# jabhinav/RetinaNet-for-Table-Detection

Hardware: AMD Instinct MI355X
Metric: images/sec RetinaNet R50-FPN 800x1333 inference (higher is better)
Workload: dtype bf16; 1 GPU; ResNet50-FPN RetinaNet inference 800x1333 bf16 batch 8/GPU incl. decode+NMS (BASELINE.json configs[1]); batch_per_gpu=8, anchors_per_image=200700, parallelism=dp1 (images sharded, no collective), batches_in_flight=2

## Files before the change

retinanet-for-table-detection_amd/csrc/rtn_conv_halo8.hip:

```cpp
#include "rtn_internal.h"
#include "rtn_device.h"
#include "rtn_conv_epilogue.h"

#ifndef RTN_H8_ABLATE
#define RTN_H8_ABLATE 0
#endif

namespace {

#ifdef RTN_H8_STAMP
__device__ unsigned long long g_h8_stamps[2][64];
#define H8_STAMP(K_)                                                                                 \
    if (stamp_on) {                                                                                  \
        unsigned long long t_;                                                                       \
        asm volatile("s_memtime %0\n\ts_waitcnt lgkmcnt(0)" : "=s"(t_) :: "memory");                 \
        if (lane == 0 && stamp_n < 64) g_h8_stamps[grp][stamp_n] = t_;                               \
        ++stamp_n;                                                                                   \
    }
#else
#define H8_STAMP(K_)
#endif

typedef __attribute__((ext_vector_type(8))) __bf16 bf16x8;
typedef __attribute__((ext_vector_type(4))) float f32x4;

constexpr unsigned OOB = 0xFFFFFF00u;
constexpr int H8_THREADS = 512;
constexpr int H8_LDS = 160 * 1024;
constexpr unsigned B_STAGE = 32768, A_BASE = 3 * 32768, A_TOGGLE = 0x18000u ^ 0x20000u;

struct H8Group {
    const char* in;
    char* out;
    const char* res;
    const char* mask;
    unsigned in_bytes, out_bytes, res_bytes, mask_bytes;
    int Hin, Win, M, tile_begin;
    int in_row_stride_b;
    int in_img_pad_b;
    float inv_cells, inv_w;
};

struct H8Params {
    H8Group g[RTN_MAX_GROUPS];
    const char* w;
    const float* bias;
    unsigned w_bytes;
    int ngroups, ntiles;
    int N, Kbytes, KH, nchunk, pad_t, pad_l, relu, out_ld, pix_b;
    int res_ld, mask_ld, mask_pre;
    int ncb, S, gps, nitems, xcd;
    int kh_fast;
    float* slab;
    unsigned slab_slice_bytes;
    int slab_ld;
    float acc_scale, out_scale;
    int out_fp8;
};

typedef int i32x8 __attribute__((ext_vector_type(8)));
__device__ __forceinline__ void mma_fp8(f32x4& acc, const uint4& a0, const uint4& a1, const uint4& b0, const uint4& b1) {
    const i32x8 A = __builtin_shufflevector(__builtin_bit_cast(i32x4, a0), __builtin_bit_cast(i32x4, a1), 0, 1, 2, 3, 4, 5, 6, 7);
    const i32x8 B = __builtin_shufflevector(__builtin_bit_cast(i32x4, b0), __builtin_bit_cast(i32x4, b1), 0, 1, 2, 3, 4, 5, 6, 7);
    acc = __builtin_amdgcn_mfma_scale_f32_16x16x128_f8f6f4(A, B, acc, 0, 0, 0, 0x7f7f7f7f, 0, 0x7f7f7f7f);
}

template <int KW, int MI, bool STAGGER, int EPI, bool SPLIT, int NW = 8, int ES = 2>
__global__ __launch_bounds__(H8_THREADS, 2) void conv_halo8_kernel(const H8Params p) {
    static_assert(NW == 8 || (NW == 4 && !SPLIT), "the half-width instance: no column blocks / K slices");
    static_assert(ES == 2 || (ES == 1 && NW == 8 && EPI == 0 && !SPLIT), "the fp8 instance: full width, plain epilogue");
    constexpr int NBP = NW / 2;
    constexpr int R = 64 * MI;
    constexpr int TM = R - KW;
    constexpr unsigned ZERO_ROW = (unsigned)(R - 1) * 128u;
    extern __shared__ __attribute__((aligned(16))) char lds[];

    const int t = threadIdx.x, lane = t & 63;
    const int wave = __builtin_amdgcn_readfirstlane(t >> 6);
    const int grp = wave >> 2;
#ifdef RTN_H8_STAMP
    bool stamp_on = false, first_item = true;
    int stamp_n = 0;
#endif
    const int wm = wave >> 1, wn = wave & 1;
    const int lr = lane >> 3, sc = (lane & 7) ^ lr;
    const int lrow = lane & 15, kq = lane >> 4;
    const unsigned lds_base = (unsigned)(size_t)(__attribute__((address_space(3))) char*)lds;

    const int G = p.KH * p.nchunk;
    const int nchunk = p.nchunk;
    const i32x4 w_srd = make_srd(p.w, p.w_bytes);

    unsigned wrow_off[NBP];
#pragma unroll
    for (int d = 0; d < NBP; ++d) {
        const int P = d * 64 + wave * 8 + lr;
        const int nrow = NW == 8 ? (P >> 7) * 128 + 8 * (P & 15) + ((P >> 4) & 7) : (P >> 6) * 64 + 4 * (P & 15) + ((P >> 4) & 3);
        wrow_off[d] = (unsigned)nrow * (unsigned)p.Kbytes + (unsigned)sc * 16u;
    }
    const unsigned b_lane = (unsigned)((wn * (16 * NW) + lrow) * 128 + ((kq ^ (lrow & 7)) << 4));


    unsigned hbase[MI];
    int hiy[MI];
    i32x4 in_srd = w_srd;
    int st_Hin = 1, st_row_b = 0;
    auto stage_tile = [&](int T) {
        if (T >= p.ntiles) {
#pragma unroll
            for (int i = 0; i < MI; ++i) { hiy[i] = -(1 << 28); hbase[i] = 0; }
            return;
        }
        int gi = 0;
#pragma unroll
        for (int i = 1; i < RTN_MAX_GROUPS; ++i)
            if (i < p.ngroups && T >= p.g[i].tile_begin) gi = i;

        const H8Group& Gs = p.g[gi];
        const int m0 = (T - Gs.tile_begin) * TM;
        const int cells = Gs.Hin * Gs.Win;
        in_srd = make_srd(Gs.in, Gs.in_bytes);
        st_Hin = Gs.Hin;
        st_row_b = Gs.in_row_stride_b;
#pragma unroll
        for (int i = 0; i < MI; ++i) {
            const int h = (i * 8 + wave) * 8 + lr;
            const int f = m0 + h - p.pad_l;
            if (h < R - 1 && f >= 0 && f < Gs.M) {
                int b, rem, y, x;
                divmod24(f, cells, Gs.inv_cells, b, rem);
                divmod24(rem, Gs.Win, Gs.inv_w, y, x);
                hiy[i] = y;
                hbase[i] = (unsigned)f * (unsigned)p.pix_b + (unsigned)b * (unsigned)Gs.in_img_pad_b + (unsigned)sc * 16u;
            } else {
                hiy[i] = -(1 << 28);
                hbase[i] = 0;
            }
        }
    };
    auto stage_a = [&](int i, int kh, int cc, unsigned abuf_addr) {
        const int dy = kh - p.pad_t;
        const unsigned delta = (unsigned)(dy * st_row_b + cc * 128);
        const bool ok = (unsigned)(hiy[i] + dy) < (unsigned)st_Hin;
#if !(RTN_H8_ABLATE & 2)
        dma16(in_srd, ok ? hbase[i] + delta : OOB, 0u, lds_base + abuf_addr + (unsigned)(wave * 1024 + i * 8192));
#endif
    };
    auto stage_b = [&](int d, unsigned kcol, int bst) {
#if !(RTN_H8_ABLATE & 1)
        dma16(w_srd, wrow_off[d], kcol, lds_base + (unsigned)bst * B_STAGE + (unsigned)(wave * 1024 + d * 8192));
#endif
    };

    unsigned a_cur = A_BASE;
    unsigned arow[KW][MI];
    auto compute_tile = [&](int T, int& gi_out, int& m0_out) {
        int gi = 0;
#pragma unroll
        for (int i = 1; i < RTN_MAX_GROUPS; ++i)
            if (i < p.ngroups && T >= p.g[i].tile_begin) gi = i;
        const H8Group& Gc = p.g[gi];
        const int m0 = (T - Gc.tile_begin) * TM;
        const int cells = Gc.Hin * Gc.Win;
        gi_out = gi;
        m0_out = m0;
#pragma unroll
        for (int i = 0; i < MI; ++i) {
            const int rloc = wm * (16 * MI) + i * 16 + lrow;
            const int m = m0 + rloc;
            const int mc = m < Gc.M ? m : Gc.M - 1;
            int b, rem, y, x;
            divmod24(mc, cells, Gc.inv_cells, b, rem);
            divmod24(rem, Gc.Win, Gc.inv_w, y, x);
#pragma unroll
            for (int kw = 0; kw < KW; ++kw) {
                const int rr = rloc + kw;
                const bool off = rloc >= TM || (unsigned)(x + kw - p.pad_l) >= (unsigned)Gc.Win;
                arow[kw][i] = a_cur + (off ? ZERO_ROW : (unsigned)(rr * 128 + ((kq ^ (rr & 7)) << 4)));
            }
        }
    };

    f32x4 acc[MI][NW];
    float bias8[8];
#pragma unroll
    for (int j = 0; j < 8; ++j) bias8[j] = 0.f;
    if (!SPLIT && p.bias && wn * (16 * NW) + NW * lrow < p.N) {
        const float4 b0 = *reinterpret_cast<const float4*>(p.bias + wn * (16 * NW) + NW * lrow);
        bias8[0] = b0.x; bias8[1] = b0.y; bias8[2] = b0.z; bias8[3] = b0.w;
        if (NW == 8) {
            const float4 b1 = *reinterpret_cast<const float4*>(p.bias + wn * 128 + 8 * lrow + 4);
            bias8[4] = b1.x; bias8[5] = b1.y; bias8[6] = b1.z; bias8[7] = b1.w;
        }
    }

    auto item_of = [&](int v) {
        if (v >= p.nitems || !p.xcd) return v;
        const int x = v & 7, j = v >> 3, base = p.nitems >> 3, rem = p.nitems & 7;
        return x * base + (x < rem ? x : rem) + j;
    };
    auto item_decode = [&](int it, int& rt, int& cb, int& sl, unsigned& cboff, int& kh0, int& cc0) {
        if (!SPLIT || it >= p.nitems) { rt = it >= p.nitems ? p.ntiles : it; cb = 0; sl = 0; cboff = 0u; kh0 = 0; cc0 = 0; return; }
        const int per = p.ncb * p.S;
        rt = it / per;
        const int rem = it - rt * per;
        cb = rem / p.S;
        sl = rem - cb * p.S;
        cboff = (unsigned)cb * 256u * (unsigned)p.Kbytes;
        const int g0 = sl * p.gps;
        if (p.kh_fast) { cc0 = g0 / p.KH; kh0 = g0 - cc0 * p.KH; }
        else { kh0 = g0 / nchunk; cc0 = g0 - kh0 * nchunk; }
    };
    const int gps = SPLIT ? p.gps : G;

    int vidx = blockIdx.x;
    int rt, cb, sl, kh0, cc0;
    unsigned cboff;
    item_decode(item_of(vidx), rt, cb, sl, cboff, kh0, cc0);
    stage_tile(rt);
#pragma unroll
    for (int i = 0; i < MI; ++i) stage_a(i, kh0, cc0, A_BASE);
    {
        const unsigned kc0 = cboff + (unsigned)((kh0 * KW * nchunk + cc0) * 128);
#pragma unroll
        for (int d = 0; d < NBP; ++d) stage_b(d, kc0, 0);
#pragma unroll
        for (int d = 0; d < NBP - 1; ++d) stage_b(d, kc0 + (unsigned)(nchunk * 128), 1);
    }
    if (NW == 8) asm volatile("s_waitcnt vmcnt(3)" ::: "memory");
    else         asm volatile("s_waitcnt vmcnt(1)" ::: "memory");
    if (STAGGER && grp == 1) __builtin_amdgcn_s_barrier();
    __builtin_amdgcn_s_barrier();


#if RTN_H8_ABLATE & 8
#define H8_LDA(KWI, KS)                                                                              \
    _Pragma("unroll") for (int i_ = 0; i_ < MI; ++i_)                                                \
        asm volatile("" : "=v"(fa[i_].x), "=v"(fa[i_].y), "=v"(fa[i_].z), "=v"(fa[i_].w));
#define H8_LDB(KWI, KS, HALF)                                                                        \
    _Pragma("unroll") for (int j_ = 0; j_ < 4; ++j_)                                                 \
        asm volatile("" : "=v"(fb[j_].x), "=v"(fb[j_].y), "=v"(fb[j_].z), "=v"(fb[j_].w));
#else
#define H8_LDA(KWI, KS)                                                                              \
    _Pragma("unroll") for (int i_ = 0; i_ < MI; ++i_)                                                \
        fa[i_] = *reinterpret_cast<const uint4*>(lds + (arow[KWI][i_] ^ ((KS) * 64u)));
#define H8_LDB(KWI, KS, HALF)                                                                        \
    _Pragma("unroll") for (int j_ = 0; j_ < 4; ++j_)                                                 \
        fb[j_] = *reinterpret_cast<const uint4*>(lds + (b_lane ^ ((KS) * 64u)) + (KWI) * B_STAGE + ((HALF) * 4 + j_) * 2048);
#endif
#if RTN_H8_ABLATE & 4
#define H8_MMA(I_, J_, HALF) asm volatile("" :: "v"(fa[I_].x), "v"(fa[I_].w), "v"(fb[J_].x), "v"(fb[J_].w));
#else
#define H8_MMA(I_, J_, HALF)                                                                         \
    acc[I_][(HALF) * 4 + J_] = __builtin_amdgcn_mfma_f32_16x16x32_bf16(                              \
        __builtin_bit_cast(bf16x8, fa[I_]), __builtin_bit_cast(bf16x8, fb[J_]), acc[I_][(HALF) * 4 + J_], 0, 0, 0);
#endif
#define H8_MFMA(HALF)                                                                                \
    H8_STAMP(1)                                                                                      \
    __builtin_amdgcn_s_barrier();                                                                    \
    H8_STAMP(2)                                                                                      \
    __builtin_amdgcn_sched_barrier(0);                                                               \
    __builtin_amdgcn_s_setprio(1);                                                                   \
    _Pragma("unroll") for (int j_ = 0; j_ < 4; ++j_)                                                 \
        _Pragma("unroll") for (int i_ = 0; i_ < MI; ++i_)                                            \
            H8_MMA(i_, j_, HALF)                                                                     \
    __builtin_amdgcn_s_setprio(0);                                                                   \
    __builtin_amdgcn_sched_barrier(0);                                                               \
    H8_STAMP(3)                                                                                      \
    __builtin_amdgcn_s_barrier();                                                                    \
    H8_STAMP(4)
#define H8_STEP(KWI)                                                                                 \
    {                                                                                                \
        const unsigned kc_n1 = (KWI) + 1 < KW ? kcol_g + ((KWI) + 1) * kw_stride : kcol_g1;          \
        const unsigned kc_n2 = (KWI) + 2 < KW ? kcol_g + ((KWI) + 2) * kw_stride : kcol_g1 + ((KWI) + 2 - KW) * kw_stride; \
        uint4 fa[MI], fb[4];                                                                         \
                                                                                        \
        H8_LDA(KWI, 0) H8_LDB(KWI, 0, 0)                                                             \
        stage_b(3, kc_n1, ((KWI) + 1) % 3);                                                          \
        H8_MFMA(0)                                                                                   \
                                                                                        \
        H8_LDB(KWI, 0, 1)                                                                            \
        stage_b(0, kc_n2, ((KWI) + 2) % 3);                                                          \
        if (2 * (KWI) < MI && (KWI) < 2) stage_a(2 * (KWI), kh1, cc1, a_cur ^ A_TOGGLE);                 \
        H8_MFMA(1)                                                                                   \
                                                                                        \
        H8_LDA(KWI, 1) H8_LDB(KWI, 1, 0)                                                             \
        stage_b(1, kc_n2, ((KWI) + 2) % 3);                                                          \
        H8_MFMA(0)                                                                                   \
                                                                                        \
        H8_LDB(KWI, 1, 1)                                                                            \
        stage_b(2, kc_n2, ((KWI) + 2) % 3);                                                          \
        if (2 * (KWI) + 1 < MI && (KWI) < 2) stage_a(2 * (KWI) + 1, kh1, cc1, a_cur ^ A_TOGGLE);         \
         \
        {                                                                                            \
            constexpr int na_ = (KWI) < 2 ? ((2 * (KWI) < MI) + (2 * (KWI) + 1 < MI)) : 0;           \
            if (na_ == 2)      asm volatile("s_waitcnt vmcnt(5)" ::: "memory");                      \
            else if (na_ == 1) asm volatile("s_waitcnt vmcnt(4)" ::: "memory");                      \
            else               asm volatile("s_waitcnt vmcnt(3)" ::: "memory");                      \
        }                                                                                            \
        H8_MFMA(1)                                                                                   \
    }
#define H8_MFMA8(HALF)                                                                               \
    __builtin_amdgcn_s_barrier();                                                                    \
    __builtin_amdgcn_sched_barrier(0);                                                               \
    __builtin_amdgcn_s_setprio(1);                                                                   \
    _Pragma("unroll") for (int j_ = 0; j_ < 4; ++j_)                                                 \
        _Pragma("unroll") for (int i_ = 0; i_ < MI; ++i_)                                            \
            mma_fp8(acc[i_][(HALF) * 4 + j_], fa[i_], fa1[i_], fb[j_], fb1[j_]);                      \
    __builtin_amdgcn_s_setprio(0);                                                                   \
    __builtin_amdgcn_sched_barrier(0);                                                               \
    __builtin_amdgcn_s_barrier();
#define H8_STEP8F(KWI)                                                                               \
    {                                                                                                \
        const unsigned kc_n1 = (KWI) + 1 < KW ? kcol_g + ((KWI) + 1) * kw_stride : kcol_g1;          \
        const unsigned kc_n2 = (KWI) + 2 < KW ? kcol_g + ((KWI) + 2) * kw_stride : kcol_g1 + ((KWI) + 2 - KW) * kw_stride; \
        uint4 fa[MI], fa1[MI], fb[4], fb1[4];                                                        \
        H8_LDA(KWI, 0)                                                                               \
        _Pragma("unroll") for (int i_ = 0; i_ < MI; ++i_)                                            \
            fa1[i_] = *reinterpret_cast<const uint4*>(lds + (arow[KWI][i_] ^ 64u));                  \
        H8_LDB(KWI, 0, 0)                                                                            \
        _Pragma("unroll") for (int j_ = 0; j_ < 4; ++j_)                                             \
            fb1[j_] = *reinterpret_cast<const uint4*>(lds + (b_lane ^ 64u) + (KWI) * B_STAGE + j_ * 2048); \
        stage_b(3, kc_n1, ((KWI) + 1) % 3);                                                          \
        if (2 * (KWI) < MI && (KWI) < 2) stage_a(2 * (KWI), kh1, cc1, a_cur ^ A_TOGGLE);             \
        H8_MFMA8(0)                                                                                  \
        H8_LDB(KWI, 0, 1)                                                                            \
        _Pragma("unroll") for (int j_ = 0; j_ < 4; ++j_)                                             \
            fb1[j_] = *reinterpret_cast<const uint4*>(lds + (b_lane ^ 64u) + (KWI) * B_STAGE + (4 + j_) * 2048); \
        stage_b(0, kc_n2, ((KWI) + 2) % 3);                                                          \
        stage_b(1, kc_n2, ((KWI) + 2) % 3);                                                          \
        stage_b(2, kc_n2, ((KWI) + 2) % 3);                                                          \
        if (2 * (KWI) + 1 < MI && (KWI) < 2) stage_a(2 * (KWI) + 1, kh1, cc1, a_cur ^ A_TOGGLE);     \
        {                                                                                            \
            constexpr int na_ = (KWI) < 2 ? ((2 * (KWI) < MI) + (2 * (KWI) + 1 < MI)) : 0;           \
            if (na_ == 2)      asm volatile("s_waitcnt vmcnt(5)" ::: "memory");                      \
            else if (na_ == 1) asm volatile("s_waitcnt vmcnt(4)" ::: "memory");                      \
            else               asm volatile("s_waitcnt vmcnt(3)" ::: "memory");                      \
        }                                                                                            \
        H8_MFMA8(1)                                                                                  \
    }
#define H8_STEP4(KWI)                                                                                \
    {                                                                                                \
        const unsigned kc_n1 = (KWI) + 1 < KW ? kcol_g + ((KWI) + 1) * kw_stride : kcol_g1;          \
        const unsigned kc_n2 = (KWI) + 2 < KW ? kcol_g + ((KWI) + 2) * kw_stride : kcol_g1 + ((KWI) + 2 - KW) * kw_stride; \
        uint4 fa[MI], fb[4];                                                                         \
        H8_LDA(KWI, 0) H8_LDB(KWI, 0, 0)                                                             \
        stage_b(1, kc_n1, ((KWI) + 1) % 3);                                                          \
        if (2 * (KWI) < MI && (KWI) < 2) stage_a(2 * (KWI), kh1, cc1, a_cur ^ A_TOGGLE);             \
        H8_MFMA(0)                                                                                   \
        H8_LDA(KWI, 1) H8_LDB(KWI, 1, 0)                                                             \
        stage_b(0, kc_n2, ((KWI) + 2) % 3);                                                          \
        if (2 * (KWI) + 1 < MI && (KWI) < 2) stage_a(2 * (KWI) + 1, kh1, cc1, a_cur ^ A_TOGGLE);     \
        {                                                                                            \
            constexpr int na_ = (KWI) < 2 ? ((2 * (KWI) < MI) + (2 * (KWI) + 1 < MI)) : 0;           \
            if (na_ == 2)      asm volatile("s_waitcnt vmcnt(3)" ::: "memory");                      \
            else if (na_ == 1) asm volatile("s_waitcnt vmcnt(2)" ::: "memory");                      \
            else               asm volatile("s_waitcnt vmcnt(1)" ::: "memory");                      \
        }                                                                                            \
        H8_MFMA(0)                                                                                   \
    }
    static_assert(KW == 3 && MI >= 2 && MI <= 4, "the B ring (3 stages) and the halo piece slots are laid out for KW = 3, MI <= 4");

    const unsigned kw_stride = (unsigned)(nchunk * 128);
    while (rt < p.ntiles) {
        int gi, m0;
        compute_tile(rt, gi, m0);
#pragma unroll
        for (int i = 0; i < MI; ++i)
#pragma unroll
            for (int j = 0; j < NW; ++j) acc[i][j] = (SPLIT || ES == 1) ? (f32x4){0.f, 0.f, 0.f, 0.f} : (f32x4){bias8[j], bias8[j], bias8[j], bias8[j]};
        int kh = kh0, cc = cc0;
        int rt1 = rt, cb1 = cb, sl1 = sl;
        unsigned cboff1 = cboff;
#pragma unroll 1
        for (int g = 0; g < gps; ++g) {
            int kh1 = kh, cc1 = cc;
            if (p.kh_fast) { if (++kh1 == p.KH) { kh1 = 0; ++cc1; } }
            else if (++cc1 == nchunk) { cc1 = 0; ++kh1; }
            if (g + 1 == gps) {
                vidx += (int)gridDim.x;
                item_decode(item_of(vidx), rt1, cb1, sl1, cboff1, kh1, cc1);
                stage_tile(rt1);
            }
#ifdef RTN_H8_STAMP
            stamp_on = blockIdx.x == 0 && (wave & 3) == 0 && first_item && g == 4;
#endif
            const unsigned kcol_g = cboff + (unsigned)((kh * KW * nchunk + cc) * 128);
            const unsigned kcol_g1 = cboff1 + (unsigned)((kh1 * KW * nchunk + cc1) * 128);
            if constexpr (ES == 1) {
                H8_STEP8F(0)
                H8_STEP8F(1)
                H8_STEP8F(2)
            } else if constexpr (NW == 8) {
                H8_STEP(0)
                H8_STEP(1)
                H8_STEP(2)
            } else {
                H8_STEP4(0)
                H8_STEP4(1)
                H8_STEP4(2)
            }
#pragma unroll
            for (int kw = 0; kw < KW; ++kw)
#pragma unroll
                for (int i = 0; i < MI; ++i) arow[kw][i] ^= A_TOGGLE;
            a_cur ^= A_TOGGLE;
            kh = kh1; cc = cc1;
        }
        kh0 = kh; cc0 = cc;
        if constexpr (ES == 1) {
            const H8Group& Gc = p.g[gi];
            const __amdgpu_buffer_rsrc_t out_rsrc = epi_rsrc(Gc.out, Gc.out_bytes);
            const int ncol = wn * 128 + 8 * lrow;
            const bool col_ok = ncol < p.N;
#pragma unroll
            for (int i = 0; i < MI; ++i)
#pragma unroll
                for (int r = 0; r < 4; ++r) {
                    const int rloc = wm * (16 * MI) + i * 16 + kq * 4 + r;
                    const int m = m0 + rloc;
                    const bool ok = col_ok && rloc < TM && m < Gc.M;
                    float v[8];
#pragma unroll
                    for (int j = 0; j < 8; ++j) {
                        v[j] = acc[i][j][r] * p.acc_scale + bias8[j];
                        if (p.relu) v[j] = v[j] > 0.f ? v[j] : 0.f;
                    }
                    if (p.out_fp8) epi_store8(epi_quant_fp8(v, p.out_scale), out_rsrc, ok ? (unsigned)m * (unsigned)p.out_ld + (unsigned)ncol : OOB);
                    else epi_store_bf16<8>(v, out_rsrc, ok ? ((unsigned)m * (unsigned)p.out_ld + (unsigned)ncol) * 2u : OOB);
                }
        } else if (SPLIT && p.S > 1) {
            const __amdgpu_buffer_rsrc_t slab_rsrc = epi_rsrc((char*)p.slab + (size_t)sl * p.slab_slice_bytes, p.slab_slice_bytes);
            const int gcol = cb * 256 + wn * 128 + 8 * lrow;
            const int Mg = p.g[gi].M;
#pragma unroll
            for (int i = 0; i < MI; ++i)
#pragma unroll
                for (int r = 0; r < 4; ++r) {
                    const int rloc = wm * (16 * MI) + i * 16 + kq * 4 + r;
                    const int m = m0 + rloc;
                    const bool ok = gcol < p.slab_ld && rloc < TM && m < Mg;
                    const unsigned off = ok ? ((unsigned)m * (unsigned)p.slab_ld + (unsigned)gcol) * 4u : OOB;
                    epi_store_f32x8<0>(acc[i], r, slab_rsrc, off, ok ? off + 16u : OOB);
                }
        } else {
            const H8Group& Gc = p.g[gi];
            const __amdgpu_buffer_rsrc_t out_rsrc = epi_rsrc(Gc.out, Gc.out_bytes);
            const __amdgpu_buffer_rsrc_t res_rsrc = epi_rsrc(Gc.res, Gc.res_bytes, EPI & 1, Gc.out);
            const __amdgpu_buffer_rsrc_t mask_rsrc = epi_rsrc(Gc.mask, Gc.mask_bytes, EPI & 2, Gc.out);
            const int ncol = (SPLIT ? cb * 256 : 0) + wn * (16 * NW) + NW * lrow;
            const bool col_ok = ncol < p.N;
            float bias_e[8];
#pragma unroll
            for (int j = 0; j < 8; ++j) bias_e[j] = 0.f;
            if (SPLIT && p.bias && col_ok) {
                const float4 b0 = *reinterpret_cast<const float4*>(p.bias + ncol);
                const float4 b1 = *reinterpret_cast<const float4*>(p.bias + ncol + 4);
                bias_e[0] = b0.x; bias_e[1] = b0.y; bias_e[2] = b0.z; bias_e[3] = b0.w;
                bias_e[4] = b1.x; bias_e[5] = b1.y; bias_e[6] = b1.z; bias_e[7] = b1.w;
            }
            constexpr int EDEPTH = NW == 8 && (EPI == 3 || (EPI == 1 && MI == 4)) ? 2 : MI;
            u32x4 rq[EDEPTH][4], mq[EDEPTH][4];
            const unsigned res_ld = (unsigned)p.res_ld, mask_ld = (unsigned)p.mask_ld;
#pragma unroll
            for (int f = 0; f < MI + EDEPTH - 1; ++f) {
                if (EPI && f < MI) {
#pragma unroll
                    for (int r = 0; r < 4; ++r) {
                        const int rloc = wm * (16 * MI) + f * 16 + kq * 4 + r;
                        const int m = m0 + rloc;
                        const bool ok = col_ok && rloc < TM && m < Gc.M;
                        if (EPI & 1) rq[f % EDEPTH][r] = epi_load_row<NW>(res_rsrc, ok ? ((unsigned)m * res_ld + (unsigned)ncol) * 2u : OOB);
                        if (EPI & 2) mq[f % EDEPTH][r] = epi_load_row<NW>(mask_rsrc, ok ? ((unsigned)m * mask_ld + (unsigned)ncol) * 2u : OOB);
                    }
                }
                const int i = f - (EDEPTH - 1);
                if (i < 0) continue;
#pragma unroll
                for (int r = 0; r < 4; ++r) {
                    const int rloc = wm * (16 * MI) + i * 16 + kq * 4 + r;
                    const int m = m0 + rloc;
                    const bool ok = col_ok && rloc < TM && m < Gc.M;
                    const unsigned off = ok ? ((unsigned)m * (unsigned)p.out_ld + (unsigned)ncol) * 2u : OOB;
                    float v[NW];
#pragma unroll
                    for (int j = 0; j < NW; ++j) v[j] = NW == 8 ? acc[i][j][r] + (SPLIT ? bias_e[j] : 0.f) : acc[i][j][r];
                    if (EPI) epi_mask_res<NW, EPI>(v, rq[i % EDEPTH][r], mq[i % EDEPTH][r], p.mask_pre);
                    if (p.relu) epi_relu(v);
                    epi_store_bf16<NW>(v, out_rsrc, off);
                }
            }
        }
        rt = rt1; cb = cb1; sl = sl1; cboff = cboff1;
#ifdef RTN_H8_STAMP
        first_item = false;
#endif
    }
#undef H8_STEP4
#undef H8_STEP8F
#undef H8_MFMA8
#undef H8_STEP
#undef H8_MFMA
#undef H8_MMA
#undef H8_LDB
#undef H8_LDA
    asm volatile("s_waitcnt vmcnt(0)" ::: "memory");
    if (STAGGER && grp == 0) __builtin_amdgcn_s_barrier();
}

template <int MI, bool ST, int EP, bool SP, int NW = 8, int ES = 2>
int h8_go(rtn_handle_t h, int grid, const H8Params& p) {
    return rtn_launch_lds<conv_halo8_kernel<3, MI, ST, EP, SP, NW, ES>>(h, dim3((unsigned)grid), dim3(H8_THREADS), H8_LDS, H8_LDS, p);
}
template <int MI>
int h8_pick(rtn_handle_t h, int grid, const H8Params& p, bool fp8, bool half, bool split, bool stagger, int epi) {
    if (fp8) return h8_go<3, true, 0, false, 8, 1>(h, grid, p);
    if (half) return rtn_with_epi<3>(epi, [&](auto e) { return h8_go<MI, true, decltype(e)::value, false, 4>(h, grid, p); });
    if (split) return h8_go<MI, true, 0, true>(h, grid, p);
    if (!stagger && epi == 0) return h8_go<MI, false, 0, false>(h, grid, p);
    return rtn_with_epi<3>(epi, [&](auto e) { return h8_go<MI, true, decltype(e)::value, false>(h, grid, p); });
}
}

int rtn_conv_halo8_try(rtn_handle_t h, const rtn_conv_desc_t* d, int grid_limit, bool stagger, bool forced, int mi_force, float* ws,
                       long long ws_cap, size_t* query, int ksplit_force, const rtn_conv_fp8_t* q8) {
    if (query) *query = 0;
    if (q8 ? d->dtype != RTN_FP8 : d->dtype != RTN_BF16) return 1;
    const int es = q8 ? 1 : 2;
    if (q8 && (query || (d->flags & ~RTN_CONV_RELU) || d->N <= 128 || d->N > 256)) return 1;
    if (d->KW != 3 || d->KH < 1 || d->KH > 7 || d->sy != 1 || d->sx != 1) return 1;
    if (d->flags & ~(RTN_CONV_RELU | RTN_CONV_RES_SAME | RTN_CONV_RELU_MASK | RTN_CONV_MASK_PRE)) return 1;
    if ((d->flags & RTN_CONV_MASK_PRE) && !(d->flags & RTN_CONV_RELU_MASK)) return 1;
    const int epi = ((d->flags & RTN_CONV_RES_SAME) ? 1 : 0) | ((d->flags & RTN_CONV_RELU_MASK) ? 2 : 0);
    const int ncb = (d->N + 255) / 256;
    if (d->N <= 64 || ncb > 8 || d->w_rows < d->N || d->N % 8 || d->out_ld % 8) return 1;
    if (ncb > 1 && epi) return 1;
    const bool half = d->N <= 128;
    if (half && !forced && rtn_env_int("RTN_CONV_H8_HALF", 1) == 0) return 1;
    if (d->Crun != d->pix_stride || (d->Crun * es) % 128 || d->Crun <= 0) return 1;
    if (d->pad_l < 0 || d->pad_l >= d->KW || d->pad_t < 0 || d->pad_t >= d->KH) return 1;
    if (((uintptr_t)d->w & 15) || ((uintptr_t)d->bias & 15)) return 1;
    const int nchunk = d->Crun * es / 128;
    const int G = d->KH * nchunk;
    const long long Kbytes = (long long)d->KH * d->KW * d->Crun * es;
    if (Kbytes * 256 * ncb >= 0xFFFFFF00ll) return 1;
    H8Params p;
    memset(&p, 0, sizeof(p));
    const int cus = h->num_cus > 0 ? h->num_cus : 256;
    long long Mtot = 0;
    for (int i = 0; i < d->ngroups; ++i) Mtot += (long long)d->g[i].Hout * d->g[i].Wout * d->batch;
    const bool can_split = !half && !q8 && d->ngroups == 1 && epi == 0 && ksplit_force != 1 && (ws_cap > 0 || query);
    const long long slab_ld = 256ll * ncb;
    int mi = 0, S = 1;
    {
        double best = 0;
        for (int cand = 4; cand >= 3; --cand) {
            if (!q8 && mi_force >= 3 && mi_force <= 4 && cand != mi_force) continue;
            if (q8 && cand == 4) continue;
            long long t = 0;
            for (int i = 0; i < d->ngroups; ++i) t += ((long long)d->g[i].Hout * d->g[i].Wout * d->batch + 64 * cand - 4) / (64 * cand - 3);
            const double step_us = 1.53 * (cand + 0.3) / 4.3;
            for (int sc = 1; sc <= 8; ++sc) {
                if (sc > 1 && (!can_split || G % sc || (ksplit_force > 1 && sc != ksplit_force))) continue;
                if (sc == 1 && ksplit_force > 1 && can_split && G % ksplit_force == 0) continue;
                if (sc > 1 && (double)sc * Mtot * slab_ld * 4 > (double)(query ? (256ll << 20) : ws_cap)) continue;
                const long long items = t * ncb * sc;
                double cost = (double)((items + cus - 1) / cus) * (3.0 * G / sc + 5.0) * step_us;
                if (sc > 1) cost += 4.0 + ((double)sc * Mtot * slab_ld * 4 + (double)Mtot * d->N * 2) / 4.0e6;
                if (mi == 0 || cost < best * 0.97) { best = cost; mi = cand; S = sc; }
            }
        }
        if (mi == 0) return 1;
    }
    if (S > 1 && !query && (!ws || ((uintptr_t)ws & 15))) return 1;
    const bool split = ncb > 1 || S > 1;
    const int TM = 64 * mi - 3;
    long long tiles = 0;
    for (int i = 0; i < d->ngroups; ++i) {
        const rtn_conv_group_t& s = d->g[i];
        if (s.Hin != s.Hout || s.Win != s.Wout || s.in_row_stride != (long long)s.Win * d->pix_stride ||
            s.in_img_stride < (long long)s.Hin * s.in_row_stride) return 1;
        if (s.in_elems < (long long)(d->batch - 1) * s.in_img_stride + (long long)s.Hin * s.in_row_stride) return 1;
        const long long cells = (long long)s.Hout * s.Wout, M = cells * d->batch;
        if (s.out_step > 1 || s.out_off != 0 || s.out_img_stride != cells * d->out_ld) return 1;
        if (M >= (1ll << 24) || M < 1) return 1;
        if (!s.in || !s.out || ((uintptr_t)s.in & 15) || ((uintptr_t)s.out & 15)) return 1;
        if (s.in_elems < M * d->Crun || s.out_elems < (M - 1) * d->out_ld + d->N) return 1;
        if (s.in_elems * 2 >= 0xFFFFFF00ll || s.out_elems * 2 >= 0xFFFFFF00ll) return 1;
        if (epi & 1) {
            if (!s.res || ((uintptr_t)s.res & 15) || s.res_ld % 8 || s.res_img_stride != cells * s.res_ld) return 1;
            if (s.res_elems < (M - 1) * s.res_ld + d->N || s.res_elems * 2 >= 0xFFFFFF00ll) return 1;
        }
        if (epi & 2) {
            if (!s.mask || ((uintptr_t)s.mask & 15) || s.mask_ld % 8 || s.mask_img_stride != cells * s.mask_ld) return 1;
            if (s.mask_elems < (M - 1) * s.mask_ld + d->N || s.mask_elems * 2 >= 0xFFFFFF00ll) return 1;
        }
        if (i > 0 && ((epi & 1) && s.res_ld != d->g[0].res_ld)) return 1;
        if (i > 0 && ((epi & 2) && s.mask_ld != d->g[0].mask_ld)) return 1;
        H8Group& g = p.g[i];
        g.res = (epi & 1) ? (const char*)s.res : nullptr;
        g.mask = (epi & 2) ? (const char*)s.mask : nullptr;
        g.res_bytes = (epi & 1) ? (unsigned)(s.res_elems * 2) : 0u;
        g.mask_bytes = (epi & 2) ? (unsigned)(s.mask_elems * 2) : 0u;
        g.in = (const char*)s.in;
        g.out = (char*)s.out;
        g.in_bytes = (unsigned)(s.in_elems * es);
        g.out_bytes = (unsigned)(s.out_elems * ((q8 && q8->out_dtype == RTN_FP8) ? 1 : 2));
        g.Hin = s.Hin; g.Win = s.Win; g.M = (int)M;
        g.tile_begin = (int)tiles;
        g.in_row_stride_b = (int)(s.in_row_stride * es);
        g.in_img_pad_b = (int)((s.in_img_stride - (long long)s.Hin * s.in_row_stride) * es);
        g.inv_cells = 1.0f / (float)cells;
        g.inv_w = 1.0f / (float)s.Win;
        tiles += (M + TM - 1) / TM;
    }
    const long long items = tiles * ncb * S;
    if (tiles < 1 || items > 0x3fffffff) return 1;
    if (!forced && items * 4 < cus) return 1;
    const long long slice_bytes = Mtot * slab_ld * 4;
    if (S > 1 && slice_bytes >= 0xFFFFFF00ll) return 1;
    if (query) { *query = S > 1 ? (size_t)(slice_bytes * S) : 0; return RTN_OK; }
    p.w = (const char*)d->w;
    p.bias = d->bias;
    p.w_bytes = (unsigned)(Kbytes * d->w_rows);
    p.ngroups = d->ngroups;
    p.ntiles = (int)tiles;
    p.N = d->N;
    p.Kbytes = (int)Kbytes;
    p.KH = d->KH;
    p.nchunk = nchunk;
    p.pad_t = d->pad_t; p.pad_l = d->pad_l;
    p.relu = (d->flags & RTN_CONV_RELU) ? 1 : 0;
    p.out_ld = d->out_ld;
    p.pix_b = d->pix_stride * es;
    if (q8) { p.acc_scale = q8->acc_scale; p.out_scale = q8->out_scale; p.out_fp8 = q8->out_dtype == RTN_FP8 ? 1 : 0; }
    p.res_ld = (epi & 1) ? d->g[0].res_ld : 0;
    p.mask_ld = (epi & 2) ? d->g[0].mask_ld : 0;
    p.mask_pre = (d->flags & RTN_CONV_MASK_PRE) ? 1 : 0;
    p.ncb = ncb; p.S = S; p.gps = G / S; p.nitems = (int)items;
    p.xcd = 1;
    p.kh_fast = 1;
    p.slab = S > 1 ? ws : nullptr;
    p.slab_slice_bytes = S > 1 ? (unsigned)slice_bytes : 0u;
    p.slab_ld = (int)slab_ld;
    int grid = cus;
    if (grid_limit > 0 && grid_limit < grid) grid = grid_limit;
    if (grid > p.nitems) grid = p.nitems;
    const int lrc = mi == 4 ? h8_pick<4>(h, grid, p, q8 != nullptr, half, split, stagger, epi)
                            : h8_pick<3>(h, grid, p, q8 != nullptr, half, split, stagger, epi);
    if (lrc != RTN_OK) return lrc;
    RTN_CHECK_LAUNCH(h, "conv_halo8_kernel");
    h->last_conv_tile = ((64 * mi) << 16) | (half ? 128 : 256);
    if (S > 1) return rtn_conv_ksplit_finish(h, ws, S, Mtot, d->N, (int)slab_ld, d->bias, p.relu, d->g[0].out, d->out_ld);
    return RTN_OK;
}

#ifdef RTN_H8_STAMP
extern "C" int rtn_debug_h8_stamps(unsigned long long* out128) {
    return (int)hipMemcpyFromSymbol(out128, HIP_SYMBOL(g_h8_stamps), sizeof(unsigned long long) * 128, 0, hipMemcpyDeviceToHost);
}
#endif
```

Measured before the change: 2420 images/sec.

## Add warp-specialized split4 halo conv kernel for half-width N tiles

Adds a new 3x3 halo conv kernel for the half-N (128 columns, MI=3) case with no fused residual or mask epilogue. Four waves act as dedicated DMA producers staging weights and halo rows into LDS, and four waves run MFMA compute with double-buffered fragments interleaved by sched_group_barrier. It is enabled by default through an environment switch. The goal is to overlap global-to-LDS transfer with matrix math instead of having every wave do both. In exchange, only half the waves issue MFMAs, the kernel relies on hand-tuned vmcnt and barrier counts, and it serves only this tile shape.

After: 2441 images/sec, median of 6. No clear change (+0.8%).

```diff
diff --git a/retinanet-for-table-detection_amd/csrc/rtn_conv_halo8.hip b/retinanet-for-table-detection_amd/csrc/rtn_conv_halo8.hip
--- a/retinanet-for-table-detection_amd/csrc/rtn_conv_halo8.hip
+++ b/retinanet-for-table-detection_amd/csrc/rtn_conv_halo8.hip
@@ -508,13 +508,289 @@
     if (STAGGER && grp == 0) __builtin_amdgcn_s_barrier();
 }
 
+__global__ __launch_bounds__(H8_THREADS, 2) void conv_halo8_split4_kernel(const H8Params p) {
+    constexpr int KW = 3, MI = 3, FM = 6, NW = 4;
+    constexpr int R = 64 * MI, TM = R - KW;
+    constexpr unsigned ZERO_ROW = (unsigned)(R - 1) * 128u;
+    extern __shared__ __attribute__((aligned(16))) char lds[];
+
+    const int t = threadIdx.x, lane = t & 63;
+    const int wave = __builtin_amdgcn_readfirstlane(t >> 6);
+    const unsigned lds_base = (unsigned)(size_t)(__attribute__((address_space(3))) char*)lds;
+    const int G = p.KH * p.nchunk, nchunk = p.nchunk;
+    const unsigned kw_stride = (unsigned)(nchunk * 128);
+    auto tile_of = [&](int v) {
+        if (v >= p.ntiles) return p.ntiles;
+        if (!p.xcd) return v;
+        const int x = v & 7, j = v >> 3, base = p.ntiles >> 3, rem = p.ntiles & 7;
+        return x * base + (x < rem ? x : rem) + j;
+    };
+    auto group_of = [&](int T) {
+        int gi = 0;
+#pragma unroll
+        for (int i = 1; i < RTN_MAX_GROUPS; ++i)
+            if (i < p.ngroups && T >= p.g[i].tile_begin) gi = i;
+        return gi;
+    };
+    const int ntile_wg = (p.ntiles - (int)blockIdx.x + (int)gridDim.x - 1) / (int)gridDim.x;
+
+    if (wave >= 4) {
+        const int sw = wave - 4;
+        const int lr = lane >> 3, sc = (lane & 7) ^ lr;
+        const i32x4 w_srd = make_srd(p.w, p.w_bytes);
+        unsigned wrow_off[2][2];
+#pragma unroll
+        for (int d = 0; d < 2; ++d)
+#pragma unroll
+            for (int u = 0; u < 2; ++u) {
+                const int P = d * 64 + (2 * sw + u) * 8 + lr;
+                const int nrow = (P >> 6) * 64 + 4 * (P & 15) + ((P >> 4) & 3);
+                wrow_off[d][u] = (unsigned)nrow * (unsigned)p.Kbytes + (unsigned)sc * 16u;
+            }
+        unsigned hbase[MI][2];
+        int hiy[MI][2];
+        const char* st_in = p.w;
+        unsigned st_in_bytes = 0;
+        int st_Hin = 1, st_row_b = 0;
+        auto stage_tile = [&](int T) {
+            if (T >= p.ntiles) {
+#pragma unroll
+                for (int i = 0; i < MI; ++i) { hiy[i][0] = hiy[i][1] = -(1 << 28); hbase[i][0] = hbase[i][1] = 0; }
+                return;
+            }
+            const H8Group& Gs = p.g[group_of(T)];
+            const int m0 = (T - Gs.tile_begin) * TM;
+            const int cells = Gs.Hin * Gs.Win;
+            st_in = Gs.in;
+            st_in_bytes = Gs.in_bytes;
+            st_Hin = Gs.Hin;
+            st_row_b = Gs.in_row_stride_b;
+#pragma unroll
+            for (int i = 0; i < MI; ++i)
+#pragma unroll
+                for (int u = 0; u < 2; ++u) {
+                    const int h = (i * 8 + 2 * sw + u) * 8 + lr;
+                    const int f = m0 + h - p.pad_l;
+                    if (h < R - 1 && f >= 0 && f < Gs.M) {
+                        int b, rem, y, x;
+                        divmod24(f, cells, Gs.inv_cells, b, rem);
+                        divmod24(rem, Gs.Win, Gs.inv_w, y, x);
+                        hiy[i][u] = y;
+                        hbase[i][u] = (unsigned)f * (unsigned)p.pix_b + (unsigned)b * (unsigned)Gs.in_img_pad_b + (unsigned)sc * 16u;
+                    } else {
+                        hiy[i][u] = -(1 << 28);
+                        hbase[i][u] = 0;
+                    }
+                }
+        };
+        int hv = blockIdx.x, hkh = 0, hcc = 0;
+        unsigned hbuf = A_BASE;
+        int bkh = 0, bcc = 0;
+        struct Cur { int kh, cc; bool left; };
+        auto next_group = [&](int kh, int cc) {
+            if (p.kh_fast) { if (++kh == p.KH) { kh = 0; ++cc; } }
+            else if (++cc == nchunk) { cc = 0; ++kh; }
+            const bool left = p.kh_fast ? cc == nchunk : kh == p.KH;
+            return Cur{left ? 0 : kh, left ? 0 : cc, left};
+        };
+        auto stage_halo = [&]() {
+            const int dy = hkh - p.pad_t;
+            const unsigned delta = (unsigned)(dy * st_row_b + hcc * 128);
+            const i32x4 srd = make_srd(st_in, st_in_bytes);
+#pragma unroll
+            for (int i = 0; i < MI; ++i)
+#pragma unroll
+                for (int u = 0; u < 2; ++u) {
+                    const bool ok = (unsigned)(hiy[i][u] + dy) < (unsigned)st_Hin;
+#if !(RTN_H8_ABLATE & 2)
+                    dma16_uniform(srd, ok ? hbase[i][u] + delta : OOB, 0u, lds_base + hbuf + (unsigned)((2 * sw + u) * 1024 + i * 8192));
+#endif
+                }
+            hbuf ^= A_TOGGLE;
+            const Cur n = next_group(hkh, hcc);
+            hkh = n.kh; hcc = n.cc;
+            if (n.left) { hv += (int)gridDim.x; stage_tile(tile_of(hv)); }
+        };
+        auto stage_b = [&](int kw) {
+            const unsigned kcol = (unsigned)__builtin_amdgcn_readfirstlane((int)((unsigned)((bkh * KW * nchunk + bcc) * 128) + (unsigned)kw * kw_stride));
+#pragma unroll
+            for (int d = 0; d < 2; ++d)
+#pragma unroll
+                for (int u = 0; u < 2; ++u) {
+#if !(RTN_H8_ABLATE & 1)
+                    dma16_uniform(w_srd, wrow_off[d][u], kcol, lds_base + (unsigned)kw * B_STAGE + (unsigned)((2 * sw + u) * 1024 + d * 8192));
+#endif
+                }
+        };
+        stage_tile(tile_of(hv));
+        stage_halo();
+        stage_b(0);
+        stage_b(1);
+        stage_b(2);
+        { const Cur n = next_group(bkh, bcc); bkh = n.kh; bcc = n.cc; }
+        stage_halo();
+        asm volatile("s_waitcnt vmcnt(14)" ::: "memory");
+        __builtin_amdgcn_s_barrier();
+#pragma unroll 1
+        for (int g = ntile_wg * G; g > 0; --g) {
+            asm volatile("s_waitcnt vmcnt(10)" ::: "memory");
+            __builtin_amdgcn_s_barrier();
+            stage_b(0);
+            asm volatile("s_waitcnt vmcnt(10)" ::: "memory");
+            __builtin_amdgcn_s_barrier();
+            stage_b(1);
+            asm volatile("s_waitcnt vmcnt(4)" ::: "memory");
+            __builtin_amdgcn_s_barrier();
+            stage_b(2);
+            { const Cur n = next_group(bkh, bcc); bkh = n.kh; bcc = n.cc; }
+            stage_halo();
+        }
+        asm volatile("s_waitcnt vmcnt(0)" ::: "memory");
+        return;
+    }
+
+    const int wm = wave >> 1, wn = wave & 1;
+    const int lrow = lane & 15, kq = lane >> 4;
+    const unsigned b_lane = (unsigned)((wn * 64 + lrow) * 128 + ((kq ^ (lrow & 7)) << 4));
+    unsigned a_cur = A_BASE;
+    unsigned arow[KW][FM];
+    auto compute_tile = [&](int T, int& gi_out, int& m0_out) {
+        const int gi = group_of(T);
+        const H8Group& Gc = p.g[gi];
+        const int m0 = (T - Gc.tile_begin) * TM;
+        const int cells = Gc.Hin * Gc.Win;
+        gi_out = gi;
+        m0_out = m0;
+        int row0 = wm * (16 * FM) + lrow;
+        asm volatile("" : "+v"(row0));
+#pragma unroll
+        for (int i = 0; i < FM; ++i) {
+            const int rloc = row0 + i * 16;
+            const int m = m0 + rloc;
+            const int mc = m < Gc.M ? m : Gc.M - 1;
+            int b, rem, y, x;
+            divmod24(mc, cells, Gc.inv_cells, b, rem);
+            divmod24(rem, Gc.Win, Gc.inv_w, y, x);
+#pragma unroll
+            for (int kw = 0; kw < KW; ++kw) {
+                const int rr = rloc + kw;
+                const bool off = rloc >= TM || (unsigned)(x + kw - p.pad_l) >= (unsigned)Gc.Win;
+                arow[kw][i] = a_cur + (off ? ZERO_ROW : (unsigned)(rr * 128 + ((kq ^ (rr & 7)) << 4)));
+            }
+        }
+    };
+    float bias4[NW];
+#pragma unroll
+    for (int j = 0; j < NW; ++j) bias4[j] = 0.f;
+    if (p.bias && wn * 64 + NW * lrow < p.N) {
+        const float4 b0 = *reinterpret_cast<const float4*>(p.bias + wn * 64 + NW * lrow);
+        bias4[0] = b0.x; bias4[1] = b0.y; bias4[2] = b0.z; bias4[3] = b0.w;
+    }
+    f32x4 acc[FM][NW];
+    uint4 fa0[FM], fb0[NW], fa1[FM], fb1[NW];
+
+#define S4_LOAD(FA, FB, AR, AX, KWI, KS)                                                             \
+    _Pragma("unroll") for (int j_ = 0; j_ < NW; ++j_)                                                \
+        FB[j_] = *reinterpret_cast<const uint4*>(lds + (b_lane ^ ((KS) * 64u)) + (KWI) * B_STAGE + j_ * 2048); \
+    _Pragma("unroll") for (int i_ = 0; i_ < FM; ++i_)                                                \
+        FA[i_] = *reinterpret_cast<const uint4*>(lds + (AR[i_] ^ ((AX) | ((KS) * 64u))));
+#if RTN_H8_ABLATE & 4
+#define S4_MMA(FA, FB)                                                                               \
+    _Pragma("unroll") for (int j_ = 0; j_ < NW; ++j_)                                                \
+        _Pragma("unroll") for (int i_ = 0; i_ < FM; ++i_)                                            \
+            asm volatile("" :: "v"(FA[i_].x), "v"(FA[i_].w), "v"(FB[j_].x), "v"(FB[j_].w));
+#else
+#define S4_MMA(FA, FB)                                                                               \
+    _Pragma("unroll") for (int j_ = 0; j_ < NW; ++j_)                                                \
+        _Pragma("unroll") for (int i_ = 0; i_ < FM; ++i_)                                            \
+            acc[i_][j_] = __builtin_amdgcn_mfma_f32_16x16x32_bf16(__builtin_bit_cast(bf16x8, FA[i_]), __builtin_bit_cast(bf16x8, FB[j_]), \
+                                                                  acc[i_][j_], 0, 0, 0);
+#endif
+#define S4_WEAVE()                                                                                   \
+    _Pragma("unroll") for (int k_ = 0; k_ < 10; ++k_) {                                              \
+        __builtin_amdgcn_sched_group_barrier(0x100, 1, 0);                                           \
+        __builtin_amdgcn_sched_group_barrier(0x008, 2, 0);                                           \
+    }                                                                                                \
+    __builtin_amdgcn_sched_group_barrier(0x008, 4, 0);
+#define S4_STEP(KWI, NKW, NAR, NAX)                                                                  \
+    __builtin_amdgcn_sched_barrier(0);                                                               \
+    S4_LOAD(fa1, fb1, arow[KWI], 0u, KWI, 1)                                                         \
+    S4_MMA(fa0, fb0)                                                                                 \
+    S4_WEAVE()                                                                                       \
+    __builtin_amdgcn_sched_barrier(0);                                                               \
+    asm volatile("s_waitcnt lgkmcnt(0)" ::: "memory");                                               \
+    __builtin_amdgcn_s_barrier();                                                                    \
+    asm volatile("" ::: "memory");                                                                   \
+    __builtin_amdgcn_sched_barrier(0);                                                               \
+    S4_LOAD(fa0, fb0, NAR, NAX, NKW, 0)                                                              \
+    S4_MMA(fa1, fb1)                                                                                 \
+    S4_WEAVE()                                                                                       \
+    __builtin_amdgcn_sched_barrier(0);
+
+    int v = blockIdx.x;
+    int rt = tile_of(v);
+    __builtin_amdgcn_s_barrier();
+    asm volatile("" ::: "memory");
+    while (rt < p.ntiles) {
+        int gi, m0;
+        compute_tile(rt, gi, m0);
+#pragma unroll
+        for (int i = 0; i < FM; ++i)
+#pragma unroll
+            for (int j = 0; j < NW; ++j) acc[i][j] = (f32x4){bias4[j], bias4[j], bias4[j], bias4[j]};
+        S4_LOAD(fa0, fb0, arow[0], 0u, 0, 0)
+#pragma unroll 1
+        for (int g = 0; g < G; ++g) {
+            S4_STEP(0, 1, arow[1], 0u)
+            S4_STEP(1, 2, arow[2], 0u)
+            S4_STEP(2, 0, arow[0], A_TOGGLE)
+#pragma unroll
+            for (int kw = 0; kw < KW; ++kw)
+#pragma unroll
+                for (int i = 0; i < FM; ++i) arow[kw][i] ^= A_TOGGLE;
+            a_cur ^= A_TOGGLE;
+        }
+        {
+            const H8Group& Gc = p.g[gi];
+            const __amdgpu_buffer_rsrc_t out_rsrc = epi_rsrc(Gc.out, Gc.out_bytes);
+            const int ncol = wn * 64 + NW * lrow;
+            const int Mg = Gc.M, relu = p.relu;
+            const unsigned out_ld2 = (unsigned)p.out_ld * 2u, col2 = (unsigned)ncol * 2u;
+            const int row_end = ncol < p.N ? (TM < Mg - m0 ? TM : Mg - m0) : 0;
+            int erow0 = wm * (16 * FM) + kq * 4;
+            asm volatile("" : "+v"(erow0));
+            const unsigned off0 = (unsigned)(m0 + erow0) * out_ld2 + col2;
+#pragma unroll
+            for (int i = 0; i < FM; ++i)
+#pragma unroll
+                for (int r = 0; r < 4; ++r) {
+                    const unsigned off = erow0 + i * 16 + r < row_end ? off0 + (unsigned)(i * 16 + r) * out_ld2 : OOB;
+                    float vv[NW];
+#pragma unroll
+                    for (int j = 0; j < NW; ++j) vv[j] = acc[i][j][r];
+                    if (relu) epi_relu(vv);
+                    epi_store_bf16<NW>(vv, out_rsrc, off);
+                }
+        }
+        v += (int)gridDim.x;
+        rt = tile_of(v);
+    }
+#undef S4_STEP
+#undef S4_WEAVE
+#undef S4_MMA
+#undef S4_LOAD
+}
+
 template <int MI, bool ST, int EP, bool SP, int NW = 8, int ES = 2>
 int h8_go(rtn_handle_t h, int grid, const H8Params& p) {
     return rtn_launch_lds<conv_halo8_kernel<3, MI, ST, EP, SP, NW, ES>>(h, dim3((unsigned)grid), dim3(H8_THREADS), H8_LDS, H8_LDS, p);
 }
 template <int MI>
-int h8_pick(rtn_handle_t h, int grid, const H8Params& p, bool fp8, bool half, bool split, bool stagger, int epi) {
+int h8_pick(rtn_handle_t h, int grid, const H8Params& p, bool fp8, bool half, bool split, bool stagger, int epi, bool split4) {
     if (fp8) return h8_go<3, true, 0, false, 8, 1>(h, grid, p);
+    if constexpr (MI == 3)
+        if (half && split4 && epi == 0)
+            return rtn_launch_lds<conv_halo8_split4_kernel>(h, dim3((unsigned)grid), dim3(H8_THREADS), H8_LDS, H8_LDS, p);
     if (half) return rtn_with_epi<3>(epi, [&](auto e) { return h8_go<MI, true, decltype(e)::value, false, 4>(h, grid, p); });
     if (split) return h8_go<MI, true, 0, true>(h, grid, p);
     if (!stagger && epi == 0) return h8_go<MI, false, 0, false>(h, grid, p);
@@ -646,8 +922,9 @@
     int grid = cus;
     if (grid_limit > 0 && grid_limit < grid) grid = grid_limit;
     if (grid > p.nitems) grid = p.nitems;
-    const int lrc = mi == 4 ? h8_pick<4>(h, grid, p, q8 != nullptr, half, split, stagger, epi)
-                            : h8_pick<3>(h, grid, p, q8 != nullptr, half, split, stagger, epi);
+    const bool split4 = half && mi == 3 && rtn_env_int("RTN_CONV_H8_NW4_SPLIT", 1) != 0;
+    const int lrc = mi == 4 ? h8_pick<4>(h, grid, p, q8 != nullptr, half, split, stagger, epi, false)
+                            : h8_pick<3>(h, grid, p, q8 != nullptr, half, split, stagger, epi, split4);
     if (lrc != RTN_OK) return lrc;
     RTN_CHECK_LAUNCH(h, "conv_halo8_kernel");
     h->last_conv_tile = ((64 * mi) << 16) | (half ? 128 : 256);
```
